# alpc91/SGRL

Hardware: AMD Instinct MI355X
Metric: env-steps/sec (whole node) + SET-actor fwd us/step, 3d_walker mix @8192 envs/GPU (higher is better)
Workload: dtype f64 (dynamics) / f32 (SET actor, obs); 1 GPU; 3D_Walker++ 8 variants x 1024 envs per GPU (config 3), random U(-1,1) actions, auto-reset, SET actor forward on every step, random-init weights; envs_per_gpu=8192, obs_max_len=287, action_max_len=21, replay_gather=none (single rank)

## Files before the change

### sgrl_amd/csrc/set_actor.hip

```cpp
#include <hip/hip_runtime.h>

#include <algorithm>
#include <cmath>
#include <cstdint>
#include <cstdlib>
#include <cstring>
#include <string>
#include <type_traits>
#include <vector>

#include "../../include/sgrl.h"
#include "../../include/sgrl_set.h"
#include "../../include/sgrl_train.h"
#include "gemm_f32.h"
#include "chain_f16.h"
#include "stream_pick.h"

namespace {

thread_local std::string g_set_err;
int sfail(int code, const std::string& msg) { g_set_err = msg; return code; }
#define SHIP_TRY(expr)                                                                     \
  do {                                                                                     \
    hipError_t _e = (expr);                                                                \
// ... 109 lines not shown
    switch (sg.kind) {
      case SGRL_PACK_COPY:
        if (i < sg.a) v = s0[i] * sg.scale;
        break;
      case SGRL_PACK_PADCOL: {
        const int r = i / sg.b, c = i % sg.b;
        if (c < sg.a) v = s0[(size_t)r * sg.a + c];
        break;
      }
      case SGRL_PACK_FOLD: {
        const int r = i / GK, k = i % GK;
        const unsigned short t = tri[k];
        if (t != 0xFFFF) {
          const int aa = t >> 8, bb = t & 255;
          const float* row = s0 + (size_t)r * (ZD * ZD);
          v = (aa == bb) ? row[aa * ZD + bb] : row[aa * ZD + bb] + row[bb * ZD + aa];
        }
        break;
      }
      case SGRL_PACK_STACK: {
        const int r = i / sg.b, c = i % sg.b;
        if (c < sg.a) {
          if (r < 30) v = s0[r * sg.a + c];
          else if (s1 && r >= 32 && r < 62) v = s1[(r - 32) * sg.a + c];
        }
        break;
      }
      case SGRL_PACK_MATMUL: {
        const int r = i / sg.b, c = i % sg.b;
        const float* ar = s0 + (size_t)r * sg.lda;
        float acc = 0.f;
        int k = 0;
        for (; k + 8 <= sg.a; k += 8) {
          float x[8], y[8];
#pragma unroll
          for (int u = 0; u < 8; u++) { x[u] = ar[k + u]; y[u] = s1[(size_t)(k + u) * sg.ldb + c]; }
#pragma unroll
          for (int u = 0; u < 8; u++) acc += x[u] * y[u];
        }
        for (; k < sg.a; k++) acc += ar[k] * s1[(size_t)k * sg.ldb + c];
        v = acc * sg.scale;
        break;
      }
      case SGRL_PACK_PERM32: {
        const int r = i / sg.a, k = i % sg.a;
        v = s0[(size_t)((r & 31) * 32 + (r >> 5)) * sg.a + k];
        break;
      }
      case SGRL_PACK_SUBMAT: {
        const int r = i / sg.b, c = i % sg.b;
        v = s0[(size_t)r * sg.lda + c];
        break;
      }
      default: break;
    }
    w[sg.dst + i] = v;
  }
}

__global__ void k_relbias(const float* rel, const float* Wr, const float* br, float* relb, const int32_t* m_off,
                          const int32_t* m_L, int n_morph) {
  const int k = blockIdx.x;
  if (k >= n_morph) return;
  const int L = m_L[k], off = m_off[k];
  for (int i = threadIdx.x; i < 2 * L * L; i += blockDim.x) {
    const int h = i / (L * L), ij = i % (L * L);
    const float* r = rel + (size_t)(off / 2) * 3 + ij * 3;
    relb[off + i] = Wr[h * 3] * r[0] + Wr[h * 3 + 1] * r[1] + Wr[h * 3 + 2] * r[2] + br[h];
  }
}

struct EnvTab {
  const int32_t* env_off;
  const int32_t* env_L;
  const int32_t* env_relb;
};
__global__ __launch_bounds__(256) void k_attention(const float* __restrict__ qkv, const float* __restrict__ U,
                                                   const float* __restrict__ gdir, const float* relb, EnvTab et,
                                                   int use_bias, const float* __restrict__ b_ng, const float* __restrict__ GD,
                                                   float* delta_dbg, float* g1, float* ng, int ng_ld,
                                                   const float* __restrict__ ln_w, const float* __restrict__ ln_b) {
  constexpr int LMAX = 14;
  __shared__ float sc[2 * LMAX * LMAX];
  __shared__ float gd[2 * LMAX * 3 * 2];
  __shared__ float dl[LMAX][128];
  const int e = blockIdx.x, t = threadIdx.x;
  const int n0 = et.env_off[e], L = et.env_L[e];
  {
    const int sub = t & 7;
    for (int idx = t >> 3; idx < 2 * L * L; idx += 32) {
      const int h = idx / (L * L), i = (idx / L) % L, j = idx % L;
      const float4* q = reinterpret_cast<const float4*>(qkv + (size_t)(n0 + i) * 768 + h * 128);
      const float4* k = reinterpret_cast<const float4*>(qkv + (size_t)(n0 + j) * 768 + 256 + h * 128);
      float s = 0.f;
#pragma unroll
      for (int u = 0; u < 4; u++) {
        const float4 a = q[sub + 8 * u], b = k[sub + 8 * u];
        s += a.x * b.x + a.y * b.y + a.z * b.z + a.w * b.w;
      }
      s += __shfl_xor(s, 1, 64); s += __shfl_xor(s, 2, 64); s += __shfl_xor(s, 4, 64);
      if (sub == 0) sc[idx] = use_bias ? s + relb[et.env_relb[e] + idx] : s;
    }
  }
  __syncthreads();
  if (t < 2 * L) {
    float* row = sc + t * L;
    float mx = row[0];
    for (int j = 1; j < L; j++) mx = fmaxf(mx, row[j]);
    float sum = 0.f;
    for (int j = 0; j < L; j++) { row[j] = expf(row[j] - mx); sum += row[j]; }
    for (int j = 0; j < L; j++) row[j] = row[j] / sum;
  }
  __syncthreads();
  for (int idx = t; idx < 2 * L * 6; idx += 256) {
    const int h = idx / (L * 6), i = (idx / 6) % L, se = idx % 6;
    const float* w = sc + (h * L + i) * L;
    float s = 0.f;
    for (int j = 0; j < L; j++) s += w[j] * gdir[(size_t)(n0 + j) * 6 + se];
    gd[idx] = s;
  }
  __syncthreads();
  {
    const int quantity = t >> 6, ln = t & 63, h = ln >> 5, c4 = (ln & 31) * 4;
    const float* vbase = quantity == 0 ? qkv + (size_t)n0 * 768 + 512 + h * 128 + c4
                                       : U + ((size_t)n0 * 3 + (quantity - 1)) * 256 + h * 128 + c4;
    auto body = [&](auto ltc, const int i0) __attribute__((always_inline)) {
      constexpr int LT = decltype(ltc)::value;
      float4 out[LT];
#pragma unroll
      for (int i = 0; i < LT; i++) out[i] = make_float4(0.f, 0.f, 0.f, 0.f);
      const float* wh = sc + h * L * L;
      if (L <= 8) {
#pragma unroll
        for (int jb = 0; jb < 8; jb += 4) {
          if (jb >= L) break;
          float4 v[4];
#pragma unroll
          for (int j = 0; j < 4; j++)
            v[j] = jb + j < L ? *reinterpret_cast<const float4*>(vbase + (size_t)(jb + j) * 768) : make_float4(0.f, 0.f, 0.f, 0.f);
#pragma unroll
          for (int j = 0; j < 4; j++)
            if (jb + j < L) {
#pragma unroll
              for (int i = 0; i < LT; i++)
                if (i0 + i < L) {
                  const float w = wh[(i0 + i) * L + jb + j];
                  out[i].x += w * v[j].x; out[i].y += w * v[j].y; out[i].z += w * v[j].z; out[i].w += w * v[j].w;
                }
            }
        }
      } else {
        float4 v = *reinterpret_cast<const float4*>(vbase);
        for (int j = 0; j < L; j++) {
          const float4 vn = *reinterpret_cast<const float4*>(vbase + (size_t)(j + 1 < L ? j + 1 : j) * 768);
#pragma unroll
          for (int i = 0; i < LT; i++)
            if (i0 + i < L) {
              const float w = wh[(i0 + i) * L + j];
              out[i].x += w * v.x; out[i].y += w * v.y; out[i].z += w * v.z; out[i].w += w * v.w;
            }
          v = vn;
        }
      }
      if (quantity != 0) {
        const float4 ga = *reinterpret_cast<const float4*>(GD + (h * 128 + c4) * 2);
        const float4 gb = *reinterpret_cast<const float4*>(GD + (h * 128 + c4) * 2 + 4);
#pragma unroll
        for (int i = 0; i < LT; i++)
          if (i0 + i < L) {
            const float* gg = gd + (h * L + i0 + i) * 6 + 2 * (quantity - 1);
            const float g0 = gg[0], g1v = gg[1];
            out[i].x += ga.x * g0 + ga.y * g1v; out[i].y += ga.z * g0 + ga.w * g1v;
            out[i].z += gb.x * g0 + gb.y * g1v; out[i].w += gb.z * g0 + gb.w * g1v;
          }
      }
      float4 bb = make_float4(0.f, 0.f, 0.f, 0.f);
      if (quantity == 0) bb = *reinterpret_cast<const float4*>(b_ng + c4);
#pragma unroll
      for (int i = 0; i < LT; i++)
        if (i0 + i < L) {
          float4 o = out[i];
          const float px = __shfl_xor(o.x, 32, 64), py = __shfl_xor(o.y, 32, 64), pz = __shfl_xor(o.z, 32, 64), pw = __shfl_xor(o.w, 32, 64);
          o = h == 0 ? make_float4(o.x + px, o.y + py, o.z + pz, o.w + pw) : make_float4(px + o.x, py + o.y, pz + o.z, pw + o.w);
          if ((i & 1) == h) {
            if (quantity != 0) {
              *reinterpret_cast<float4*>(g1 + ((size_t)(n0 + i0 + i) * 3 + (quantity - 1)) * 128 + c4) = o;
            } else {
              o.x += bb.x; o.y += bb.y; o.z += bb.z; o.w += bb.w;
              *reinterpret_cast<float4*>(&dl[i0 + i][c4]) = o;
              if (delta_dbg) *reinterpret_cast<float4*>(delta_dbg + (size_t)(n0 + i0 + i) * 128 + c4) = o;
            }
          }
        }
    };
    for (int i0 = 0; i0 < L; i0 += 4) body(std::integral_constant<int, 4>{}, i0);
  }
  __syncthreads();
  const int lane = t & 63;
  const float w0 = ln_w[lane], w1 = ln_w[64 + lane], b0 = ln_b[lane], b1 = ln_b[64 + lane];
  for (int i = t >> 6; i < L; i += 4) {
    float* row = ng + (size_t)(n0 + i) * ng_ld;
    const float v0 = row[lane] + dl[i][lane], v1 = row[64 + lane] + dl[i][64 + lane];
    const float mu = wave_sum_f32(v0 + v1) * (1.f / 128.f);
    const float d0 = v0 - mu, d1 = v1 - mu;
    const float var = wave_sum_f32(d0 * d0 + d1 * d1) * (1.f / 128.f);
    const float inv = 1.0f / sqrtf(var + 1e-5f);
    row[lane] = d0 * inv * w0 + b0;
    row[64 + lane] = d1 * inv * w1 + b1;
  }
}

__global__ __launch_bounds__(256) void k_add_ln(const float* x, int ldx, const float* delta, int ldd, const float* w,
                                                const float* b, float* out1, int ld1, float* out2, int ld2, int N) {
  const int row = blockIdx.x * 4 + (threadIdx.x >> 6), lane = threadIdx.x & 63;
  if (row >= N) return;
  float v0 = x[(size_t)row * ldx + lane], v1 = x[(size_t)row * ldx + 64 + lane];
  if (delta) { v0 += delta[(size_t)row * ldd + lane]; v1 += delta[(size_t)row * ldd + 64 + lane]; }
  const float mu = wave_sum_f32(v0 + v1) * (1.f / 128.f);
  const float d0 = v0 - mu, d1 = v1 - mu;
  const float var = wave_sum_f32(d0 * d0 + d1 * d1) * (1.f / 128.f);
  const float inv = 1.0f / sqrtf(var + 1e-5f);
  const float y0 = d0 * inv * w[lane] + b[lane], y1 = d1 * inv * w[64 + lane] + b[64 + lane];
  if (out1) { out1[(size_t)row * ld1 + lane] = y0; out1[(size_t)row * ld1 + 64 + lane] = y1; }
  if (out2) { out2[(size_t)row * ld2 + lane] = y0; out2[(size_t)row * ld2 + 64 + lane] = y1; }
}

__global__ __launch_bounds__(128) void k_equiv(const float* __restrict__ T, const float* __restrict__ W5,
                                               const float* __restrict__ g1, float* g, float* outg, int N) {
  __shared__ float Ts[8 * 96];
  const int t = threadIdx.x, n0 = blockIdx.x * 8;
  const int rows = min(8, N - n0) * 3;
  for (int o = t; o < 8 * 96; o += 128) Ts[o] = (n0 + o / 96 < N) ? T[(size_t)n0 * 96 + o] : 0.f;
  float w[32];
#pragma unroll
  for (int c = 0; c < 32; c++) w[c] = W5[t * 32 + c];
  __syncthreads();
#pragma unroll
  for (int rb = 0; rb < 24; rb += 8) {
    if (rb >= rows) break;
    float gv[8], g1v[8];
#pragma unroll
    for (int r = 0; r < 8; r++) {
      const size_t row = (size_t)n0 * 3 + (rb + r < rows ? rb + r : 0);
      gv[r] = g[row * D + t];
      g1v[r] = g1[row * D + t];
    }
#pragma unroll
    for (int r = 0; r < 8; r++) {
      if (rb + r >= rows) break;
      const float* tt = Ts + (rb + r) * 32;
      float v = 0.f;
#pragma unroll
      for (int c = 0; c < 32; c++) v += tt[c] * w[c];
      const size_t row = (size_t)n0 * 3 + rb + r;
      const float gn = gv[r] + (g1v[r] + v);
      g[row * D + t] = gn;
      if (outg) {
        outg[row * OGLD + 8 + t] = gn;
        if (t < OGLD - 136) outg[row * OGLD + 136 + t] = 0.f;
      }
    }
  }
}

__global__ __launch_bounds__(128) void k_head_out(const float* __restrict__ T, const float* __restrict__ wdec,
                                                  const float* __restrict__ obs, int obs_ld, NodeTab nt, float* act, int act_ld,
                                                  float max_action, int N) {
  const int n = blockIdx.x * 4 + (threadIdx.x >> 5), c = threadIdx.x & 31;
  if (n >= N) return;
  float vec[3];
  const float wd = wdec[c];
  for (int s = 0; s < 3; s++) {
    float v = T[(size_t)n * 96 + s * 32 + c] * wd;
    for (int off = 16; off > 0; off >>= 1) v += __shfl_xor(v, off, 32);
    vec[s] = v;
  }
  if (c < 3) {
    const int env = nt.node_env[n], limb = nt.node_limb[n];
    const float* o = obs + (size_t)env * obs_ld + 41 * limb + 3 * (5 + c);
    const float a = o[0] * vec[0] + o[1] * vec[1] + o[2] * vec[2];
    act[(size_t)env * act_ld + 3 * limb + c] = max_action * tanhf(a);
  }
}


__global__ __launch_bounds__(128) void k_head_out2(const float* __restrict__ m2, const float* __restrict__ z, const float* __restrict__ obs,
                                                   int obs_ld, NodeTab nt, float* act, int act_ld, float max_action, int N) {
  const int n = blockIdx.x * 4 + (threadIdx.x >> 5), c = threadIdx.x & 31;
  if (n >= N) return;
  float vec[3];
  const float mq = m2[(size_t)n * 32 + c];
  for (int s = 0; s < 3; s++) {
    float v = z[(size_t)n * 96 + s * 32 + c] * mq;
    for (int off = 16; off > 0; off >>= 1) v += __shfl_xor(v, off, 32);
    vec[s] = v;
  }
  if (c < 3) {
    const int env = nt.node_env[n], limb = nt.node_limb[n];
    const float* o = obs + (size_t)env * obs_ld + 41 * limb + 3 * (5 + c);
    const float a = o[0] * vec[0] + o[1] * vec[1] + o[2] * vec[2];
    act[(size_t)env * act_ld + 3 * limb + c] = max_action * tanhf(a);
  }
}

__global__ __launch_bounds__(256) void k_q_head(const float* __restrict__ c, const float* __restrict__ w, const float* __restrict__ b,
                                                const float* __restrict__ fn, NodeTab nt, float* q, int q_ld, int N) {
  const int n = blockIdx.x * 4 + (threadIdx.x >> 6), lane = threadIdx.x & 63;
  if (n >= N) return;
  const float* row = c + (size_t)n * 256;
  float v = row[lane] * w[lane] + row[64 + lane] * w[64 + lane] + row[128 + lane] * w[128 + lane] + row[192 + lane] * w[192 + lane];
  v = wave_sum_f32(v);
  if (lane == 0) q[(size_t)nt.node_env[n] * q_ld + nt.node_limb[n]] = (v + b[0]) / fn[n];
}

}

struct GraphCfg {
  std::vector<int32_t> key_i;
  std::vector<float> key_f;
  int n_env = 0, N = 0, n_morph = 0, TM = 0, Lmax = 0;
  int split_env = 0, split_node = 0;
  int32_t *d_node_env = nullptr, *d_node_limb = nullptr, *d_node_mnode = nullptr, *d_trav = nullptr;
  int32_t *d_env_off = nullptr, *d_env_L = nullptr, *d_env_relb = nullptr, *d_m_off = nullptr, *d_m_L = nullptr;
  float *d_rel = nullptr, *d_relb = nullptr;
  uint64_t last_use = 0;
  void release() {
    void* ptrs[] = {d_node_env, d_node_limb, d_node_mnode, d_trav, d_env_off, d_env_L, d_env_relb, d_m_off, d_m_L, d_rel, d_relb};
    for (void* q : ptrs) if (q) (void)hipFree(q);
  }
};

struct sgrl_set {
  const float* w = nullptr;
  int64_t off[SGRL_SET_NW];
  bool have_w = false, have_graph = false;
  int n_env = 0, N = 0, n_morph = 0, TM = 0, Lmax = 0;
  int split_env = 0, split_node = 0;
  int last_split = 0;
  int32_t *d_node_env = nullptr, *d_node_limb = nullptr, *d_node_mnode = nullptr, *d_trav = nullptr;
  int32_t *d_env_off = nullptr, *d_env_L = nullptr, *d_env_relb = nullptr, *d_m_off = nullptr, *d_m_L = nullptr;
  float *d_rel = nullptr, *d_relb = nullptr;
  std::vector<GraphCfg*> cfgs;
  uint64_t use_clock = 0;
  int64_t generation = 0;
  float* ws = nullptr;
  int64_t ws_floats = 0;
  int carved_N = 0;
  float* cat_cur = nullptr;
  float *g, *cat, *cat2, *zc, *fn, *h256, *qkv, *vg, *g1, *z2, *mat, *t256, *t256b, *t128a, *t128b, *delta,
      *outg, *outng, *gdir;
  float* wstack = nullptr;
  const float* site_ptr[SGRL_SET_NSITES];
  bool hold = false, packed_ok = false;
  int packed_form = 0;
  hipEvent_t ev_pack = nullptr;
  const float* l2mf_w = nullptr;
  const float* l2mf_b = nullptr;
  unsigned short* d_tri = nullptr;
  bool stack_dirty = true;
  bool stack_critic = false;
  int stop_after = -1;
  int small_nodes = -1;
  int gemm_form = 0;
  sgrl_gemm::EncMat* d_enc = nullptr;
  int n_enc = 0, enc_rows = 0;
  float* wsc = nullptr;
  std::vector<std::pair<int64_t, int>> enc_index;
  bool live = false;
  float* wflat = nullptr;
  unsigned* wwords = nullptr;
  int64_t wflat_floats = 0;
  sgrl_pack_seg* d_segs = nullptr;
  int2* d_chunks = nullptr;
  int n_chunks = 0;
  hipStream_t side = nullptr;
  hipEvent_t ev_fork = nullptr, ev_join = nullptr, ev_l3 = nullptr;
  hipEvent_t ev_fork_b = nullptr, ev_join_b = nullptr, ev_split = nullptr, ev_merge = nullptr;
  std::vector<hipStream_t> side_ok_for;
  int side_picks = 0;
  const float* W(int slot) const { return w + off[slot]; }
  const float* WL(int layer, int k) const { return w + off[SGRL_SET_NGLOBAL + layer * SGRL_SET_NLAYER + k]; }
};

namespace {

constexpr int64_t kPerNodeFloats = 384  + 256 + 256  + 96  + 1  + 256  + 768  +
                                   768  + 384  + 96  + 96  + 256 + 256  +
                                   128 + 128 + 128  + 3 * OGLD  + 160  + 6 ;
constexpr int kWsArrays = 19;

int64_t ws_floats_for(int64_t N) { return kPerNodeFloats * N + 32 * kWsArrays; }

void free_graphs(sgrl_set* s) {
  for (GraphCfg* c : s->cfgs) { c->release(); delete c; }
  s->cfgs.clear();
  if (s->ws) (void)hipFree(s->ws);
  s->ws = nullptr; s->ws_floats = 0; s->carved_N = 0;
  s->have_graph = false;
}

template <class T>
int upload(T** dst, const std::vector<T>& v) {
  if (hipMalloc(dst, sizeof(T) * (v.size() ? v.size() : 1)) != hipSuccess) return -1;
  if (!v.empty() && hipMemcpy(*dst, v.data(), sizeof(T) * v.size(), hipMemcpyHostToDevice) != hipSuccess) return -1;
  return 0;
}

void pick_split(const std::vector<int32_t>& env_off, int N, int* env_out, int* node_out) {
  int best = 0, best_rank = -1;
  int64_t best_dist = 0;
  for (size_t e = 1; e < env_off.size(); e++) {
    const int n = env_off[e];
    const int64_t dist = std::abs(2 * (int64_t)n - N);
    const int rank = 2 * dist > N / 16 ? 0 : (n % 128 == 0 ? 3 : n % 64 == 0 ? 2 : 1);
    if (best_rank < 0 || rank > best_rank || (rank == best_rank && dist < best_dist)) { best = (int)e; best_rank = rank; best_dist = dist; }
  }
  *env_out = best;
  *node_out = best ? env_off[best] : 0;
}

int use_cfg(sgrl_set* s, GraphCfg* c) {
  const int64_t N = c->N;
  const int64_t need = ws_floats_for(N);
  if (need > s->ws_floats) {
    if (s->ws) { (void)hipFree(s->ws); s->generation++; }
    s->ws = nullptr; s->ws_floats = 0; s->carved_N = 0;
    if (hipMalloc(&s->ws, sizeof(float) * need) != hipSuccess) return sfail(SGRL_ERR_HIP, "device allocation failed (SET workspace)");
    s->ws_floats = need;
  }
  if (s->carved_N != c->N) {
    float* p = s->ws;
    auto take = [&](int64_t n) { float* r = p; p += (n + 31) & ~int64_t(31); return r; };
    s->g = take(384 * N); s->cat = take(256 * N); s->cat2 = take(256 * N); s->zc = take(96 * N); s->fn = take(N);
    s->h256 = take(256 * N); s->qkv = take(768 * N); s->vg = take(768 * N);
    s->g1 = take(384 * N); s->z2 = take(96 * N); s->mat = take(96 * N); s->t256 = take(256 * N); s->t256b = take(256 * N); s->t128a = take(128 * N);
    s->t128b = take(128 * N); s->delta = take(128 * N); s->outg = take(3 * OGLD * N); s->outng = take(160 * N); s->gdir = take(6 * N);
    if (p - s->ws > s->ws_floats) return sfail(SGRL_ERR_LIMIT, "workspace carve-up overflow");
    s->carved_N = c->N;
  }
  s->n_env = c->n_env; s->N = c->N; s->n_morph = c->n_morph; s->TM = c->TM; s->Lmax = c->Lmax;
  s->split_env = c->split_env; s->split_node = c->split_node;
  s->d_node_env = c->d_node_env; s->d_node_limb = c->d_node_limb; s->d_node_mnode = c->d_node_mnode; s->d_trav = c->d_trav;
  s->d_env_off = c->d_env_off; s->d_env_L = c->d_env_L; s->d_env_relb = c->d_env_relb; s->d_m_off = c->d_m_off; s->d_m_L = c->d_m_L;
  s->d_rel = c->d_rel; s->d_relb = c->d_relb;
  c->last_use = ++s->use_clock;
  s->have_graph = true;
  return SGRL_OK;
}

bool gemm_use_split() {
  static const bool v = [] { const char* e = getenv("SGRL_SET_GEMM"); return !(e && e[0] == 'f'); }();
  return v;
}
struct GemmCtx {
  int form = SGRL_SET_FORM_F16X3;
  const float* w_base = nullptr; const unsigned* w_words = nullptr;
  const float* wsc = nullptr;
  const std::vector<std::pair<int64_t, int>>* enc_index = nullptr;
};
thread_local GemmCtx g_gemm;
int gemm_default_form() {
  static const int v = [] { const char* e = getenv("SGRL_SET_GEMM"); return (e && e[0] == 'b') ? SGRL_SET_FORM_BF16X6 : SGRL_SET_FORM_F16X3; }();
  return v;
}
const float* wsc_of(const float* W) {
  if (!g_gemm.enc_index) return nullptr;
  const int64_t off = W - g_gemm.w_base;
  for (const auto& e : *g_gemm.enc_index) if (e.first == off) return g_gemm.wsc + e.second;
  return nullptr;
}
GemmArgs with_words(const GemmArgs& a) {
  GemmArgs b = a;
  b.W = reinterpret_cast<const float*>(g_gemm.w_words + (a.W - g_gemm.w_base));
  b.wscale = wsc_of(a.W);
  return b;
}
template <int F> struct GemmKernels {
  static constexpr auto kNarrow = k_gemm2<F, 4, 1, 1, 2, 16, 1>;
  static constexpr auto kWide = k_gemm2<F, 4, 2, 1, 2, 32, 2>;
  static constexpr auto kSquare = k_gemm2<F, 4, 4, 1, 1, 32, 2>;
  static constexpr auto kSplit = sgrl_gemm::k_gemm3<F, 4, 2, 1, 2, 16, 2>;
  static constexpr auto kSplitH = sgrl_gemm::k_gemm3<F, 4, 2, 1, 2, 16, 2, false, false, false, 0, false, 2, true, 2>;
  static constexpr int kSplitHLds = sgrl_gemm::TileCfg3<4, 2, 1, 2, 16, 2>::kLdsBytes;
  static constexpr int kNarrowLds = sgrl_gemm::TileCfg<4, 1, 1, 2, 16>::kLdsBytes;
  static constexpr int kWideLds = sgrl_gemm::TileCfg<4, 2, 1, 2, 32>::kLdsBytes;
  static constexpr int kSquareLds = sgrl_gemm::TileCfg<4, 4, 1, 1, 32>::kLdsBytes;
  static constexpr int kSplitLds = sgrl_gemm::TileCfg3<4, 2, 1, 2, 16>::kLdsBytes;
  static bool raise_lds_limits() {
    return hipFuncSetAttribute(reinterpret_cast<const void*>(kNarrow), hipFuncAttributeMaxDynamicSharedMemorySize, kNarrowLds) == hipSuccess &&
           hipFuncSetAttribute(reinterpret_cast<const void*>(kWide), hipFuncAttributeMaxDynamicSharedMemorySize, kWideLds) == hipSuccess &&
           hipFuncSetAttribute(reinterpret_cast<const void*>(kSquare), hipFuncAttributeMaxDynamicSharedMemorySize, kSquareLds) == hipSuccess &&
           hipFuncSetAttribute(reinterpret_cast<const void*>(kSplit), hipFuncAttributeMaxDynamicSharedMemorySize, kSplitLds) == hipSuccess &&
           hipFuncSetAttribute(reinterpret_cast<const void*>(kSplitH), hipFuncAttributeMaxDynamicSharedMemorySize, kSplitHLds) == hipSuccess;
  }
  static void launch(hipStream_t st, const GemmArgs& a) {
    const int tiles128 = ((a.M + 127) / 128) * ((a.N + 127) / 128);
    if (a.N <= 64 || (a.K % 32) != 0) {
      hipLaunchKernelGGL(kNarrow, dim3(((a.M + 127) / 128) * ((a.N + 63) / 64)), dim3(256), kNarrowLds, st, a);
    } else if (gemm_use_split()) {
      if (g_gemm.form == SGRL_SET_FORM_F16X3) hipLaunchKernelGGL(kSplitH, dim3(tiles128), dim3(512), kSplitHLds, st, with_words(a));
      else hipLaunchKernelGGL(kSplit, dim3(tiles128), dim3(512), kSplitLds, st, a);
    } else if (tiles128 < 512) {
      hipLaunchKernelGGL(kNarrow, dim3(((a.M + 127) / 128) * ((a.N + 63) / 64)), dim3(256), kNarrowLds, st, a);
    } else if (a.N >= 512) {
      hipLaunchKernelGGL(kWide, dim3(tiles128), dim3(512), kWideLds, st, a);
    } else {
      hipLaunchKernelGGL(kSquare, dim3(tiles128), dim3(1024), kSquareLds, st, a);
    }
  }
};

constexpr auto kProjH = sgrl_gemm::k_gemm3<EPI_ZSPLIT, 4, 1, 1, 2, 16, 2, false, false, false, 0, false, 2, false, 2>;
constexpr int kProjHLds = sgrl_gemm::TileCfg3<4, 1, 1, 2, 16, 2>::kLdsBytes;

constexpr auto kGemmEquiv = sgrl_gemm::k_gemm3<EPI_ROWDIV | EPI_EQUIV, 4, 2, 1, 2, 16, 2>;
constexpr auto kGemmEquivH = sgrl_gemm::k_gemm3<EPI_ROWDIV | EPI_EQUIV, 4, 2, 1, 2, 16, 2, false, false, false, 0, false, 2, true, 2>;
constexpr int kEquivLds = GemmKernels<0>::kSplitLds > 128 * 100 * 4 ? GemmKernels<0>::kSplitLds : 128 * 100 * 4;
int launch_gemm_equiv(hipStream_t st, const float* A, int lda, const float* W, int ldw, const float* bias, int M, int K,
                      const float* rowdiv, const float* zq, float* tout) {
  if (K % 32 != 0 || (lda & 3) || (ldw & 3)) return sfail(SGRL_ERR_ARG, "gemm_equiv: K must be a multiple of 32 and rows 16-byte aligned");
  GemmArgs a{A, lda, W, ldw, bias, nullptr, 0, M, 1024, K, EPI_ROWDIV | EPI_EQUIV, rowdiv, nullptr, 0};
  a.zq = zq; a.tout = tout;
  if (g_gemm.form == SGRL_SET_FORM_F16X3) hipLaunchKernelGGL(kGemmEquivH, dim3(((M + 127) / 128) * 8), dim3(512), kEquivLds, st, with_words(a));
  else hipLaunchKernelGGL(kGemmEquiv, dim3(((M + 127) / 128) * 8), dim3(512), kEquivLds, st, a);
  return SGRL_OK;
}

constexpr auto kGemmGram = sgrl_gemm::k_gemm3<EPI_RELU, 4, 2, 1, 2, 16, 2, false, false, false, 0, true>;
// ... 131 lines not shown
  if (!live) return;
  float ss = 0.f;
  for (int k = lane; k < GK; k += 64) {
    const unsigned t = tri[k];
    float v = 0.f;
    if (t != 0xFFFFu) {
      const int a = t >> 8, b = t & 255;
      v = zs[w][a] * zs[w][b] + zs[w][32 + a] * zs[w][32 + b] + zs[w][64 + a] * zs[w][64 + b];
      ss += (a == b ? 1.f : 2.f) * v * v;
    }
    A[(size_t)node * GK + k] = v;
  }
  ss = wave_sum_f32(ss);
  if (lane == 0) fn[node] = sqrtf(ss) + 1.f;
}

__global__ __launch_bounds__(128) void k_zmat_perm(const float* __restrict__ zq, const float* __restrict__ matp,
                                                   float* __restrict__ tout) {
  __shared__ float ms[32 * 33], zs[96];
  const int t = threadIdx.x;
  const size_t n = blockIdx.x;
  for (int o = t; o < 1024; o += 128) ms[(o >> 5) * 33 + (o & 31)] = matp[n * 1024 + o];
  if (t < 96) zs[t] = zq[n * 96 + t];
  __syncthreads();
  if (t >= 96) return;
  const int sI = t >> 5, c = t & 31;
  float acc = 0.f;
#pragma unroll
  for (int a = 0; a < 32; a++) acc += zs[sI * 32 + a] * ms[c * 33 + a];
  tout[n * 96 + t] = acc;
}

int small_fail() { return sfail(SGRL_ERR_HIP, std::string("small-batch product: ") + sgrl_train_last_error()); }

int small_gemm(hipStream_t st, const float* A, int lda, const float* W, int ldw, const float* bias, float* C, int ldc, int M,
               int N, int K, int flags = 0, const float* rowdiv = nullptr) {
  if (flags & ~(EPI_RELU | EPI_ROWDIV)) return sfail(SGRL_ERR_ARG, "small gemm: unsupported epilogue");
  const int rc = sgrl_linear_forward(A, lda, W, ldw, bias, (flags & EPI_ROWDIV) ? rowdiv : nullptr, C, ldc, M, N, K,
                                     (flags & EPI_RELU) ? 1 : 0, st);
  return rc == SGRL_OK ? rc : small_fail();
}

int run_forward(sgrl_set* s, const float* obs, int obs_ld, float* act, int act_ld, float max_action, hipStream_t st,
                bool critic = false, const float* action = nullptr, int action_ld = 0) {
  const int N = s->N, N3 = 3 * s->N;
  const int ngf = critic ? 20 : 17;
  g_gemm.form = s->gemm_form ? s->gemm_form : gemm_default_form();
  if (!s->live || !s->wwords) g_gemm.form = SGRL_SET_FORM_BF16X6;
  if (!gemm_use_split()) g_gemm.form = SGRL_SET_FORM_BF16X6;
  g_gemm.w_base = s->w;
  g_gemm.w_words = s->wwords;
  g_gemm.wsc = s->wsc;
  g_gemm.enc_index = &s->enc_index;
  NodeTab nt{s->d_node_env, s->d_node_limb, s->d_node_mnode, s->d_trav, s->TM};
  EnvTab et{s->d_env_off, s->d_env_L, s->d_env_relb};
  const bool small = N <= (s->small_nodes >= 0 ? s->small_nodes : small_nodes());
  hipStreamCaptureStatus cap = hipStreamCaptureStatusNone;
  (void)hipStreamIsCapturing(st, &cap);
  static const bool serial_env = [] { const char* e = getenv("SGRL_SET_ONE_STREAM"); return e && e[0] == '1'; }();
  const bool one_stream = small || cap != hipStreamCaptureStatusNone || serial_env;
  if (!one_stream && sgrl_streams::enabled() && s->side_picks < 6 &&
      std::find(s->side_ok_for.begin(), s->side_ok_for.end(), st) == s->side_ok_for.end()) {
    s->side_picks++;
    hipStream_t chosen = sgrl_streams::pick({st}, s->side);
    if (chosen != s->side) s->side_ok_for.clear();
    s->side = chosen;
    s->side_ok_for.push_back(st);
  }
  hipStream_t sd = one_stream ? st : s->side;
  auto fork = [&]() { if (!one_stream) { (void)hipEventRecord(s->ev_fork, st); (void)hipStreamWaitEvent(sd, s->ev_fork, 0); } };
  auto join = [&]() { if (!one_stream) { (void)hipEventRecord(s->ev_join, sd); (void)hipStreamWaitEvent(st, s->ev_join, 0); } };
  (void)hipMemsetAsync(act, 0, sizeof(float) * (size_t)s->n_env * act_ld, st);
  const bool want_words = !small && g_gemm.form == SGRL_SET_FORM_F16X3 && gemm_use_split();
  const bool reuse = s->live && s->hold && s->packed_ok && (!want_words || s->packed_form == SGRL_SET_FORM_F16X3) && cap == hipStreamCaptureStatusNone;
  if (reuse) (void)hipStreamWaitEvent(st, s->ev_pack, 0);
  if (s->live && !reuse)
    hipLaunchKernelGGL(k_pack, dim3(s->n_chunks), dim3(256), 0, st, s->d_segs, s->d_chunks, s->d_tri, s->wflat);
  const bool encode = s->live && !reuse && want_words;
  if (encode) {
    fork();
    hipLaunchKernelGGL(sgrl_gemm::k_encode_rows, dim3((s->enc_rows + 3) / 4), dim3(256), 0, sd, s->wflat, s->wwords, s->wsc, s->d_enc, s->n_enc,
                       s->enc_rows);
  }
  hipLaunchKernelGGL(k_relbias, dim3(s->n_morph), dim3(256), 0, st, s->d_rel, s->W(SGRL_SET_REL_W), s->W(SGRL_SET_REL_B),
                     s->d_relb, s->d_m_off, s->d_m_L, s->n_morph);
  hipLaunchKernelGGL(k_embed, dim3((N + kEmbedNodes - 1) / kEmbedNodes), dim3(128), 0, st, obs, obs_ld, action, action_ld, ngf, nt,
                     s->W(SGRL_SET_GENC), s->W(SGRL_SET_ENC_W), s->W(SGRL_SET_ENC_B), s->W(SGRL_SET_EMB0), s->W(SGRL_SET_EMB1),
                     s->W(SGRL_SET_EMB2), s->g, s->cat, s->outg, s->outng, s->gdir, s->zc, s->z2, N);
  if (encode) join();
  if (s->live && !reuse && cap == hipStreamCaptureStatusNone) {
    s->packed_ok = s->hold;
    s->packed_form = want_words ? SGRL_SET_FORM_F16X3 : SGRL_SET_FORM_BF16X6;
    if (s->hold) (void)hipEventRecord(s->ev_pack, st);
  }
  const bool chain = !small && chain_enabled() && gemm_use_split() && g_gemm.form == SGRL_SET_FORM_F16X3;
  constexpr bool chain_eq = false, head_fold = true, fuse_update = true;
  struct Part {
    int r0, M, e0, ne;
    hipStream_t st, sd;
    hipEvent_t ev_fork, ev_join;
    float *catc, *cato;
    hipEvent_t ev_site0;
  };
  s->cat_cur = s->cat;
  auto site_w = [&](int site) -> const float* {
    return s->live ? s->site_ptr[site] : s->wstack + (size_t)site * 64 * 128;
  };
  if (!s->live && (s->stack_dirty || s->stack_critic != critic)) {
    s->stack_critic = critic;
    auto sw = [&](int site) { return s->wstack + (size_t)site * 64 * 128; };
    for (int l = 0; l < SGRL_SET_LAYERS; l++) {
      hipLaunchKernelGGL(k_stack_proj, dim3(32), dim3(256), 0, st, s->WL(l, SGRL_SET_A_GPROJ), (const float*)nullptr, D, D, sw(2 * l));
      hipLaunchKernelGGL(k_stack_proj, dim3(32), dim3(256), 0, st, s->WL(l, SGRL_SET_F_GPROJ2), s->WL(l, SGRL_SET_F_GPROJ3), D, D, sw(2 * l + 1));
    }
    hipLaunchKernelGGL(k_stack_proj, dim3(36), dim3(256), 0, st, s->W(SGRL_SET_GGPROJ), critic ? (const float*)nullptr : s->W(SGRL_SET_GPROJ), 136, OGLD, sw(6));
    s->stack_dirty = false;
  }
  constexpr int kStages = 4 * SGRL_SET_LAYERS + 2, kStop = 1;
  auto stage = [&](Part& p, int k) -> int {
    const int N = p.M, N3 = 3 * p.M, lnb = (N + 3) / 4;
    hipStream_t st = p.st, sd = p.sd;
    const size_t r = (size_t)p.r0;
    float *const g = s->g + 384 * r, *const zc = s->zc + 96 * r, *const z2 = s->z2 + 96 * r, *const fn = s->fn + r,
          *const h256 = s->h256 + 256 * r, *const qkv = s->qkv + 768 * r, *const vg = s->vg + 768 * r, *const g1 = s->g1 + 384 * r,
          *const mat = s->mat + 96 * r, *const t256 = s->t256 + 256 * r, *const t256b = s->t256b + 256 * r,
          *const t128a = s->t128a + 128 * r, *const t128b = s->t128b + 128 * r, *const delta = s->delta + 128 * r,
          *const outg = s->outg + 3 * OGLD * r, *const outng = s->outng + 160 * r, *const cat = s->cat + 256 * r,
          *const cat2 = s->cat2 + 256 * r;
    float *const catc = p.catc + 256 * r, *const cato = p.cato + 256 * r, *const ng = catc + 128;
    const NodeTab ntp{nt.node_env + r, nt.node_limb + r, nt.node_mnode + r, nt.trav, nt.TM};
    auto fork = [&]() { if (!one_stream && sd != st) { (void)hipEventRecord(p.ev_fork, st); (void)hipStreamWaitEvent(sd, p.ev_fork, 0); } };
    auto join = [&]() { if (!one_stream && sd != st) { (void)hipEventRecord(p.ev_join, sd); (void)hipStreamWaitEvent(st, p.ev_join, 0); } };
    int rc = SGRL_OK;
    float* const scratch = qkv;
#define G(...) do { rc = small ? small_gemm(st, __VA_ARGS__) : launch_gemm(st, __VA_ARGS__); if (rc != SGRL_OK) return rc; } while (0)
    auto gram_gemm = [&](const float* W_, const float* b_, float* C_, int ldc_, int N_) -> int {
      if (!small) return launch_gemm_gram(st, zc, W_, b_, C_, ldc_, N, N_, fn);
      hipLaunchKernelGGL(k_gram576, dim3((N + 3) / 4), dim3(256), 0, st, zc, s->d_tri, scratch, fn, N);
      return small_gemm(st, scratch, GK, W_, GK, b_, C_, ldc_, N, N_, GK, EPI_RELU);
    };
    auto equiv_gemm = [&](const float* A_, const float* W_, const float* b_) -> int {
      if (!small) return launch_gemm_equiv(st, A_, 256, W_, 256, b_, N, 256, fn, z2, mat);
      const int r_ = small_gemm(st, A_, 256, W_, 256, b_, scratch, 1024, N, 1024, 256, EPI_ROWDIV, fn);
      if (r_ != SGRL_OK) return r_;
      hipLaunchKernelGGL(k_zmat_perm, dim3(N), dim3(128), 0, st, z2, scratch, mat);
      return SGRL_OK;
    };
#define GG(W_, b_, C_, ldc_, N_) do { rc = gram_gemm(W_, b_, C_, ldc_, N_); if (rc != SGRL_OK) return rc; } while (0)
    auto pg = [&](const float* X, int ldx, int K, int site, float* z2_) -> int {
      if (K % 16 != 0 || (ldx & 3)) return sfail(SGRL_ERR_ARG, "projection: K must be a multiple of 16 and rows 16-byte aligned");
      if (small) {
        int r_ = small_gemm(st, X, ldx, site_w(site), K, nullptr, zc, ZD, N3, 30, K);
        if (r_ == SGRL_OK && z2_) r_ = small_gemm(st, X, ldx, site_w(site) + (size_t)32 * K, K, nullptr, z2_, ZD, N3, 30, K);
        return r_;
      }
      GemmArgs a{X, ldx, site_w(site), K, nullptr, zc, ZD, N3, z2_ ? 64 : 32, K, EPI_ZSPLIT, nullptr, z2_, ZD};
      if (g_gemm.form == SGRL_SET_FORM_F16X3 && gemm_use_split())
        hipLaunchKernelGGL(kProjH, dim3(((a.M + 127) / 128) * ((a.N + 63) / 64)), dim3(256), kProjHLds, st, with_words(a));
      else
        GemmKernels<EPI_ZSPLIT>::launch(st, a);
      return SGRL_OK;
    };
#define PG(...) do { rc = pg(__VA_ARGS__); if (rc != SGRL_OK) return rc; } while (0)
#define GS(...) do { rc = small ? small_gemm(sd, __VA_ARGS__) : launch_gemm(sd, __VA_ARGS__); if (rc != SGRL_OK) return rc; } while (0)
    const int l = k / 4;
    if (k < 4 * SGRL_SET_LAYERS && k % 4 == 0) {
      fork();
      GS(g, D, s->WL(l, SGRL_SET_VG_W), D, nullptr, vg, 256, N3, 256, D);
      if (chain) {
        rc = launch_site(st, g, D, D, site_w(2 * l), zc, nullptr, fn, s->WL(l, SGRL_SET_A_LG1_W), s->WL(l, SGRL_SET_A_LG1_B), 256,
                         s->WL(l, SGRL_SET_A_LG2_W), s->WL(l, SGRL_SET_A_LG2_B), catc, 256, N);
        if (rc != SGRL_OK) return rc;
        if (l == 0 && p.ev_site0) (void)hipEventRecord(p.ev_site0, st);
      } else {
        PG(g, D, D, 2 * l, nullptr);
        GG(s->WL(l, SGRL_SET_A_LG1_W), s->WL(l, SGRL_SET_A_LG1_B), h256, 256, 256);
// ... 311 lines not shown
    if (hipMalloc(&s->d_enc, sizeof(sgrl_gemm::EncMat) * mats.size()) != hipSuccess || hipMalloc(&s->wsc, sizeof(float) * rows_total) != hipSuccess ||
        hipMemcpy(s->d_enc, mats.data(), sizeof(sgrl_gemm::EncMat) * mats.size(), hipMemcpyHostToDevice) != hipSuccess)
      return sfail(SGRL_ERR_HIP, "device allocation failed in sgrl_set_bind_params (row-scale table)");
  }
  s->n_chunks = (int)chunks.size();
  s->w = s->wflat;
  std::memcpy(s->off, offsets, sizeof(int64_t) * SGRL_SET_NW);
  for (int k = 0; k < SGRL_SET_NSITES; k++) s->site_ptr[k] = s->wflat + offsets[SGRL_SET_NW + k];
  {
    std::vector<int64_t> b2(offsets, offsets + n_offsets);
    b2.push_back(total_floats);
    std::sort(b2.begin(), b2.end());
    const int64_t ow = offsets[SGRL_SET_NW + SGRL_SET_NSITES], ob = offsets[SGRL_SET_NW + SGRL_SET_NSITES + 1];
    const bool have = *std::upper_bound(b2.begin(), b2.end(), ow) - ow >= 32 * 256;
    s->l2mf_w = have ? s->wflat + ow : nullptr;
    s->l2mf_b = have ? s->wflat + ob : nullptr;
  }
  s->live = true;
  s->have_w = true;
  return SGRL_OK;
}

int sgrl_set_graph(sgrl_set* s, int n_morph, const int32_t* morph_L, const int32_t* morph_count, const int32_t* trav,
                   const float* rel) {
  if (!s || n_morph <= 0 || !morph_L || !morph_count || !trav || !rel) return sfail(SGRL_ERR_ARG, "sgrl_set_graph: bad argument");
  std::vector<int32_t> key_i;
  size_t ntrav = 0, nrel = 0;
  for (int k = 0; k < n_morph; k++) {
    if (morph_L[k] < 2 || morph_L[k] > 14) return sfail(SGRL_ERR_LIMIT, "limb count must be in [2, 14]");
    if (morph_count[k] < 0) return sfail(SGRL_ERR_ARG, "negative morph_count");
    ntrav += 3 * (size_t)morph_L[k];
    nrel += 3 * (size_t)morph_L[k] * morph_L[k];
  }
  key_i.push_back(n_morph);
  key_i.insert(key_i.end(), morph_L, morph_L + n_morph);
  key_i.insert(key_i.end(), morph_count, morph_count + n_morph);
  key_i.insert(key_i.end(), trav, trav + ntrav);
  for (GraphCfg* c : s->cfgs)
    if (c->key_i == key_i && c->key_f.size() == nrel && std::memcmp(c->key_f.data(), rel, sizeof(float) * nrel) == 0)
      return use_cfg(s, c);
  std::vector<int32_t> node_env, node_limb, node_mnode, env_off, env_L, env_relb, m_off, m_L, travT;
  int TM = 0, relb_off = 0, env = 0, node = 0, Lmax = 0;
  std::vector<int> m_node0;
  for (int k = 0; k < n_morph; k++) {
    m_node0.push_back(TM);
    m_off.push_back(relb_off);
    m_L.push_back(morph_L[k]);
    TM += morph_L[k];
    relb_off += 2 * morph_L[k] * morph_L[k];
    if (morph_L[k] > Lmax) Lmax = morph_L[k];
  }
  travT.assign(3 * (size_t)TM, 0);
  {
    size_t tp = 0;
    for (int k = 0; k < n_morph; k++) {
      const int L = morph_L[k];
      for (int q = 0; q < 3; q++)
        for (int i = 0; i < L; i++) {
          const int v = trav[tp + q * L + i];
          if (v < 0 || v >= 15) return sfail(SGRL_ERR_ARG, "traversal index out of range");
          travT[(size_t)q * TM + m_node0[k] + i] = v;
        }
      tp += 3 * (size_t)L;
    }
  }
  for (int k = 0; k < n_morph; k++) {
    for (int c = 0; c < morph_count[k]; c++) {
      env_off.push_back(node);
      env_L.push_back(morph_L[k]);
      env_relb.push_back(m_off[k]);
      for (int i = 0; i < morph_L[k]; i++) {
        node_env.push_back(env);
        node_limb.push_back(i);
        node_mnode.push_back(m_node0[k] + i);
        node++;
      }
      env++;
    }
  }
  if (node == 0) return sfail(SGRL_ERR_ARG, "no environments");
  if ((int)s->cfgs.size() >= SGRL_SET_GRAPH_CACHE) {
    size_t lru = 0;
    for (size_t i = 1; i < s->cfgs.size(); i++) if (s->cfgs[i]->last_use < s->cfgs[lru]->last_use) lru = i;
    s->cfgs[lru]->release();
    s->generation++;
    delete s->cfgs[lru];
    s->cfgs.erase(s->cfgs.begin() + lru);
  }
  GraphCfg* c = new GraphCfg();
  c->key_i = std::move(key_i);
  c->key_f.assign(rel, rel + nrel);
  c->n_env = env; c->N = node; c->n_morph = n_morph; c->TM = TM; c->Lmax = Lmax;
  pick_split(env_off, node, &c->split_env, &c->split_node);
  bool ok = upload(&c->d_node_env, node_env) == 0 && upload(&c->d_node_limb, node_limb) == 0 &&
            upload(&c->d_node_mnode, node_mnode) == 0 && upload(&c->d_trav, travT) == 0 &&
            upload(&c->d_env_off, env_off) == 0 && upload(&c->d_env_L, env_L) == 0 && upload(&c->d_env_relb, env_relb) == 0 &&
            upload(&c->d_m_off, m_off) == 0 && upload(&c->d_m_L, m_L) == 0 && upload(&c->d_rel, c->key_f) == 0;
  if (ok) ok = hipMalloc(&c->d_relb, sizeof(float) * relb_off) == hipSuccess;
  if (!ok) { c->release(); delete c; return sfail(SGRL_ERR_HIP, "device allocation failed in sgrl_set_graph"); }
  s->cfgs.push_back(c);
  return use_cfg(s, c);
}

int sgrl_set_forward(sgrl_set* s, const float* obs, int obs_ld, float* act, int act_ld, float max_action, void* stream) {
  if (!s || !obs || !act) return sfail(SGRL_ERR_ARG, "sgrl_set_forward: null argument");
  if (!s->have_w || !s->have_graph) return sfail(SGRL_ERR_ARG, "sgrl_set_forward: weights or graph not set");
  if (obs_ld < 41 * s->Lmax || act_ld < 3 * s->Lmax)
    return sfail(SGRL_ERR_ARG, "sgrl_set_forward: obs_ld < 41 * Lmax or act_ld < 3 * Lmax (rows too narrow for the largest morphology)");
  return run_forward(s, obs, obs_ld, act, act_ld, max_action, (hipStream_t)stream);
}

int sgrl_set_forward_q(sgrl_set* s, const float* obs, int obs_ld, const float* action, int action_ld, float* q, int q_ld,
                       void* stream) {
  if (!s || !obs || !action || !q) return sfail(SGRL_ERR_ARG, "sgrl_set_forward_q: null argument");
  if (!s->have_w || !s->have_graph) return sfail(SGRL_ERR_ARG, "sgrl_set_forward_q: weights or graph not set");
  if (obs_ld < 41 * s->Lmax || action_ld < 3 * s->Lmax || q_ld < s->Lmax)
    return sfail(SGRL_ERR_ARG, "sgrl_set_forward_q: obs_ld < 41 * Lmax, action_ld < 3 * Lmax or q_ld < Lmax");
  return run_forward(s, obs, obs_ld, q, q_ld, 0.f, (hipStream_t)stream, true, action, action_ld);
}

int sgrl_set_time_forward(sgrl_set* s, const float* obs, int obs_ld, float* act, int act_ld, float max_action,
                          int reps, void* stream, float* ms_out) {
  if (!s || !obs || !act || !ms_out || reps <= 0) return sfail(SGRL_ERR_ARG, "sgrl_set_time_forward: bad argument");
  if (!s->have_w || !s->have_graph) return sfail(SGRL_ERR_ARG, "weights or graph not set");
  if (obs_ld < 41 * s->Lmax || act_ld < 3 * s->Lmax) return sfail(SGRL_ERR_ARG, "sgrl_set_time_forward: rows too narrow for the largest morphology");
  hipEvent_t t0, t1;
  SHIP_TRY(hipEventCreate(&t0));
  SHIP_TRY(hipEventCreate(&t1));
  SHIP_TRY(hipEventRecord(t0, (hipStream_t)stream));
  for (int r = 0; r < reps; r++) {
    int rc = run_forward(s, obs, obs_ld, act, act_ld, max_action, (hipStream_t)stream);
    if (rc != SGRL_OK) return rc;
  }
  SHIP_TRY(hipEventRecord(t1, (hipStream_t)stream));
  SHIP_TRY(hipEventSynchronize(t1));
  float ms = 0;
  SHIP_TRY(hipEventElapsedTime(&ms, t0, t1));
  (void)hipEventDestroy(t0);
  (void)hipEventDestroy(t1);
  *ms_out = ms / reps;
  return SGRL_OK;
}

int sgrl_set_hold_weights(sgrl_set* s, int hold) {
  if (!s) return sfail(SGRL_ERR_ARG, "sgrl_set_hold_weights: null handle");
  s->hold = hold != 0;
  s->packed_ok = false;
  return SGRL_OK;
}

int sgrl_set_num_nodes(const sgrl_set* s) { return s ? s->N : SGRL_ERR_ARG; }
int64_t sgrl_set_workspace_bytes(const sgrl_set* s) { return s ? s->ws_floats * 4 : -1; }
int64_t sgrl_set_generation(const sgrl_set* s) { return s ? s->generation : -1; }
int sgrl_set_last_split(const sgrl_set* s) { return s ? s->last_split : SGRL_ERR_ARG; }

int sgrl_set_peek(sgrl_set* s, int which, float* host, int64_t n_floats) {
  if (!s || !host || !s->have_graph) return sfail(SGRL_ERR_ARG, "sgrl_set_peek: bad argument");
  const float* src[] = {s->g, s->cat_cur ? s->cat_cur : s->cat, s->zc, s->fn, s->qkv, nullptr, nullptr, s->mat, s->g1, s->delta, s->outng};
  const int64_t per[] = {384, 256, 96, 1, 768, 0, 0, 96, 384, 128, 160};
  if (which < 0 || which > 10 || !src[which] || n_floats > per[which] * s->N) return sfail(SGRL_ERR_ARG, "sgrl_set_peek: bad buffer or size");
  SHIP_TRY(hipDeviceSynchronize());
  SHIP_TRY(hipMemcpy(host, src[which], sizeof(float) * n_floats, hipMemcpyDeviceToHost));
  return SGRL_OK;
}

int sgrl_set_debug_stop_after(sgrl_set* s, int stage) {
// ... 153 lines not shown
```

Baseline: 1.932 million env-steps/s.

## Prefetch attention operands into registers and cache relative-bias across packed-weight reuse

Restructures the per-env attention kernel so that the first Q/K fragments, relative bias, gdir rows, V rows (for L<=8), the GD/bias projections and the first LayerNorm rows are all loaded up front, before the barriers. This overlaps global-load latency with the score computation. gdir is staged in shared memory instead of being re-read from global in the gd reduction. Separately, the k_relbias launch is skipped when packed weights are reused and the current graph config's relb epoch matches the pack epoch. This removes one kernel launch per step, at the cost of extra register pressure and new epoch bookkeeping that could go stale.

```diff
diff --git a/sgrl_amd/csrc/set_actor.hip b/sgrl_amd/csrc/set_actor.hip
--- a/sgrl_amd/csrc/set_actor.hip
+++ b/sgrl_amd/csrc/set_actor.hip
@@ -215,27 +215,56 @@
                                                    const float* __restrict__ ln_w, const float* __restrict__ ln_b) {
   constexpr int LMAX = 14;
   __shared__ float sc[2 * LMAX * LMAX];
+  __shared__ float gs[LMAX * 6];
   __shared__ float gd[2 * LMAX * 3 * 2];
   __shared__ float dl[LMAX][128];
   const int e = blockIdx.x, t = threadIdx.x;
-  const int n0 = et.env_off[e], L = et.env_L[e];
+  const int n0 = et.env_off[e], L = et.env_L[e], rb0 = use_bias ? et.env_relb[e] : 0;
+  const int sub = t & 7, idx0 = t >> 3, lane = t & 63;
+  const int quantity = t >> 6, h = lane >> 5, c4 = (lane & 31) * 4;
+  const float* vbase = quantity == 0 ? qkv + (size_t)n0 * 768 + 512 + h * 128 + c4
+                                     : U + ((size_t)n0 * 3 + (quantity - 1)) * 256 + h * 128 + c4;
+  float4 qa[4], kb[4];
+  float rb = 0.f;
+  if (idx0 < 2 * L * L) {
+    const int hh = idx0 / (L * L), i = (idx0 / L) % L, j = idx0 % L;
+    const float4* q = reinterpret_cast<const float4*>(qkv + (size_t)(n0 + i) * 768 + hh * 128);
+    const float4* k = reinterpret_cast<const float4*>(qkv + (size_t)(n0 + j) * 768 + 256 + hh * 128);
+#pragma unroll
+    for (int u = 0; u < 4; u++) { qa[u] = q[sub + 8 * u]; kb[u] = k[sub + 8 * u]; }
+    if (use_bias) rb = relb[rb0 + idx0];
+  }
+  float gdv = 0.f;
+  if (t < 6 * L) gdv = gdir[(size_t)n0 * 6 + t];
+  float4 v8[8];
   {
-    const int sub = t & 7;
-    for (int idx = t >> 3; idx < 2 * L * L; idx += 32) {
-      const int h = idx / (L * L), i = (idx / L) % L, j = idx % L;
-      const float4* q = reinterpret_cast<const float4*>(qkv + (size_t)(n0 + i) * 768 + h * 128);
-      const float4* k = reinterpret_cast<const float4*>(qkv + (size_t)(n0 + j) * 768 + 256 + h * 128);
-      float s = 0.f;
-#pragma unroll
-      for (int u = 0; u < 4; u++) {
-        const float4 a = q[sub + 8 * u], b = k[sub + 8 * u];
-        s += a.x * b.x + a.y * b.y + a.z * b.z + a.w * b.w;
-      }
-      s += __shfl_xor(s, 1, 64); s += __shfl_xor(s, 2, 64); s += __shfl_xor(s, 4, 64);
-      if (sub == 0) sc[idx] = use_bias ? s + relb[et.env_relb[e] + idx] : s;
-    }
-  }
+    const int held = L <= 8 ? L : 1;
+#pragma unroll
+    for (int j = 0; j < 8; j++)
+      if (j < held) v8[j] = *reinterpret_cast<const float4*>(vbase + (size_t)j * 768);
+  }
+  for (int idx = idx0; idx < 2 * L * L; idx += 32) {
+    if (idx != idx0) {
+      const int hh = idx / (L * L), i = (idx / L) % L, j = idx % L;
+      const float4* q = reinterpret_cast<const float4*>(qkv + (size_t)(n0 + i) * 768 + hh * 128);
+      const float4* k = reinterpret_cast<const float4*>(qkv + (size_t)(n0 + j) * 768 + 256 + hh * 128);
+#pragma unroll
+      for (int u = 0; u < 4; u++) { qa[u] = q[sub + 8 * u]; kb[u] = k[sub + 8 * u]; }
+      if (use_bias) rb = relb[rb0 + idx];
+    }
+    float s = 0.f;
+#pragma unroll
+    for (int u = 0; u < 4; u++) {
+      const float4 a = qa[u], b = kb[u];
+      s += a.x * b.x + a.y * b.y + a.z * b.z + a.w * b.w;
+    }
+    s += __shfl_xor(s, 1, 64); s += __shfl_xor(s, 2, 64); s += __shfl_xor(s, 4, 64);
+    if (sub == 0) sc[idx] = use_bias ? s + rb : s;
+  }
+  if (t < 6 * L) gs[t] = gdv;
   __syncthreads();
+  const float4 pa = quantity == 0 ? *reinterpret_cast<const float4*>(b_ng + c4) : *reinterpret_cast<const float4*>(GD + (h * 128 + c4) * 2);
+  const float4 pb = quantity == 0 ? make_float4(0.f, 0.f, 0.f, 0.f) : *reinterpret_cast<const float4*>(GD + (h * 128 + c4) * 2 + 4);
   if (t < 2 * L) {
     float* row = sc + t * L;
     float mx = row[0];
@@ -246,71 +275,28 @@
   }
   __syncthreads();
   for (int idx = t; idx < 2 * L * 6; idx += 256) {
-    const int h = idx / (L * 6), i = (idx / 6) % L, se = idx % 6;
-    const float* w = sc + (h * L + i) * L;
+    const int hh = idx / (L * 6), i = (idx / 6) % L, se = idx % 6;
+    const float* w = sc + (hh * L + i) * L;
     float s = 0.f;
-    for (int j = 0; j < L; j++) s += w[j] * gdir[(size_t)(n0 + j) * 6 + se];
+    for (int j = 0; j < L; j++) s += w[j] * gs[j * 6 + se];
     gd[idx] = s;
   }
   __syncthreads();
   {
-    const int quantity = t >> 6, ln = t & 63, h = ln >> 5, c4 = (ln & 31) * 4;
-    const float* vbase = quantity == 0 ? qkv + (size_t)n0 * 768 + 512 + h * 128 + c4
-                                       : U + ((size_t)n0 * 3 + (quantity - 1)) * 256 + h * 128 + c4;
-    auto body = [&](auto ltc, const int i0) __attribute__((always_inline)) {
-      constexpr int LT = decltype(ltc)::value;
-      float4 out[LT];
-#pragma unroll
-      for (int i = 0; i < LT; i++) out[i] = make_float4(0.f, 0.f, 0.f, 0.f);
-      const float* wh = sc + h * L * L;
-      if (L <= 8) {
-#pragma unroll
-        for (int jb = 0; jb < 8; jb += 4) {
-          if (jb >= L) break;
-          float4 v[4];
-#pragma unroll
-          for (int j = 0; j < 4; j++)
-            v[j] = jb + j < L ? *reinterpret_cast<const float4*>(vbase + (size_t)(jb + j) * 768) : make_float4(0.f, 0.f, 0.f, 0.f);
-#pragma unroll
-          for (int j = 0; j < 4; j++)
-            if (jb + j < L) {
-#pragma unroll
-              for (int i = 0; i < LT; i++)
-                if (i0 + i < L) {
-                  const float w = wh[(i0 + i) * L + jb + j];
-                  out[i].x += w * v[j].x; out[i].y += w * v[j].y; out[i].z += w * v[j].z; out[i].w += w * v[j].w;
-                }
-            }
-        }
-      } else {
-        float4 v = *reinterpret_cast<const float4*>(vbase);
-        for (int j = 0; j < L; j++) {
-          const float4 vn = *reinterpret_cast<const float4*>(vbase + (size_t)(j + 1 < L ? j + 1 : j) * 768);
-#pragma unroll
-          for (int i = 0; i < LT; i++)
-            if (i0 + i < L) {
-              const float w = wh[(i0 + i) * L + j];
-              out[i].x += w * v.x; out[i].y += w * v.y; out[i].z += w * v.z; out[i].w += w * v.w;
-            }
-          v = vn;
-        }
-      }
+    const float* wh = sc + h * L * L;
+    auto finish = [&](float4 (&out)[4], const int i0) __attribute__((always_inline)) {
       if (quantity != 0) {
-        const float4 ga = *reinterpret_cast<const float4*>(GD + (h * 128 + c4) * 2);
-        const float4 gb = *reinterpret_cast<const float4*>(GD + (h * 128 + c4) * 2 + 4);
-#pragma unroll
-        for (int i = 0; i < LT; i++)
+#pragma unroll
+        for (int i = 0; i < 4; i++)
           if (i0 + i < L) {
             const float* gg = gd + (h * L + i0 + i) * 6 + 2 * (quantity - 1);
             const float g0 = gg[0], g1v = gg[1];
-            out[i].x += ga.x * g0 + ga.y * g1v; out[i].y += ga.z * g0 + ga.w * g1v;
-            out[i].z += gb.x * g0 + gb.y * g1v; out[i].w += gb.z * g0 + gb.w * g1v;
+            out[i].x += pa.x * g0 + pa.y * g1v; out[i].y += pa.z * g0 + pa.w * g1v;
+            out[i].z += pb.x * g0 + pb.y * g1v; out[i].w += pb.z * g0 + pb.w * g1v;
           }
       }
-      float4 bb = make_float4(0.f, 0.f, 0.f, 0.f);
-      if (quantity == 0) bb = *reinterpret_cast<const float4*>(b_ng + c4);
-#pragma unroll
-      for (int i = 0; i < LT; i++)
+#pragma unroll
+      for (int i = 0; i < 4; i++)
         if (i0 + i < L) {
           float4 o = out[i];
           const float px = __shfl_xor(o.x, 32, 64), py = __shfl_xor(o.y, 32, 64), pz = __shfl_xor(o.z, 32, 64), pw = __shfl_xor(o.w, 32, 64);
@@ -319,27 +305,75 @@
             if (quantity != 0) {
               *reinterpret_cast<float4*>(g1 + ((size_t)(n0 + i0 + i) * 3 + (quantity - 1)) * 128 + c4) = o;
             } else {
-              o.x += bb.x; o.y += bb.y; o.z += bb.z; o.w += bb.w;
+              o.x += pa.x; o.y += pa.y; o.z += pa.z; o.w += pa.w;
               *reinterpret_cast<float4*>(&dl[i0 + i][c4]) = o;
               if (delta_dbg) *reinterpret_cast<float4*>(delta_dbg + (size_t)(n0 + i0 + i) * 128 + c4) = o;
             }
           }
         }
     };
-    for (int i0 = 0; i0 < L; i0 += 4) body(std::integral_constant<int, 4>{}, i0);
+    if (L <= 8) {
+      for (int i0 = 0; i0 < L; i0 += 4) {
+        float4 out[4];
+#pragma unroll
+        for (int i = 0; i < 4; i++) out[i] = make_float4(0.f, 0.f, 0.f, 0.f);
+#pragma unroll
+        for (int j = 0; j < 8; j++)
+          if (j < L) {
+#pragma unroll
+            for (int i = 0; i < 4; i++)
+              if (i0 + i < L) {
+                const float w = wh[(i0 + i) * L + j];
+                out[i].x += w * v8[j].x; out[i].y += w * v8[j].y; out[i].z += w * v8[j].z; out[i].w += w * v8[j].w;
+              }
+          }
+        finish(out, i0);
+      }
+    } else {
+      for (int i0 = 0; i0 < L; i0 += 4) {
+        float4 out[4];
+#pragma unroll
+        for (int i = 0; i < 4; i++) out[i] = make_float4(0.f, 0.f, 0.f, 0.f);
+        float4 v = v8[0];
+        for (int j = 0; j < L; j++) {
+          const float4 vn = *reinterpret_cast<const float4*>(vbase + (size_t)(j + 1 < L ? j + 1 : j) * 768);
+#pragma unroll
+          for (int i = 0; i < 4; i++)
+            if (i0 + i < L) {
+              const float w = wh[(i0 + i) * L + j];
+              out[i].x += w * v.x; out[i].y += w * v.y; out[i].z += w * v.z; out[i].w += w * v.w;
+            }
+          v = vn;
+        }
+        finish(out, i0);
+      }
+    }
   }
   __syncthreads();
-  const int lane = t & 63;
+  float x0[2] = {0.f, 0.f}, x1[2] = {0.f, 0.f};
+#pragma unroll
+  for (int r = 0; r < 2; r++)
+    if (quantity + 4 * r < L) {
+      const float* row = ng + (size_t)(n0 + quantity + 4 * r) * ng_ld;
+      x0[r] = row[lane]; x1[r] = row[64 + lane];
+    }
   const float w0 = ln_w[lane], w1 = ln_w[64 + lane], b0 = ln_b[lane], b1 = ln_b[64 + lane];
-  for (int i = t >> 6; i < L; i += 4) {
+  auto ln_row = [&](const int i, const float xa, const float xb) __attribute__((always_inline)) {
     float* row = ng + (size_t)(n0 + i) * ng_ld;
-    const float v0 = row[lane] + dl[i][lane], v1 = row[64 + lane] + dl[i][64 + lane];
+    const float v0 = xa + dl[i][lane], v1 = xb + dl[i][64 + lane];
     const float mu = wave_sum_f32(v0 + v1) * (1.f / 128.f);
     const float d0 = v0 - mu, d1 = v1 - mu;
     const float var = wave_sum_f32(d0 * d0 + d1 * d1) * (1.f / 128.f);
     const float inv = 1.0f / sqrtf(var + 1e-5f);
     row[lane] = d0 * inv * w0 + b0;
     row[64 + lane] = d1 * inv * w1 + b1;
+  };
+#pragma unroll
+  for (int r = 0; r < 2; r++)
+    if (quantity + 4 * r < L) ln_row(quantity + 4 * r, x0[r], x1[r]);
+  for (int i = quantity + 8; i < L; i += 4) {
+    const float* row = ng + (size_t)(n0 + i) * ng_ld;
+    ln_row(i, row[lane], row[64 + lane]);
   }
 }
 
@@ -456,6 +490,7 @@
   int32_t *d_node_env = nullptr, *d_node_limb = nullptr, *d_node_mnode = nullptr, *d_trav = nullptr;
   int32_t *d_env_off = nullptr, *d_env_L = nullptr, *d_env_relb = nullptr, *d_m_off = nullptr, *d_m_L = nullptr;
   float *d_rel = nullptr, *d_relb = nullptr;
+  uint64_t relb_epoch = 0;
   uint64_t last_use = 0;
   void release() {
     void* ptrs[] = {d_node_env, d_node_limb, d_node_mnode, d_trav, d_env_off, d_env_L, d_env_relb, d_m_off, d_m_L, d_rel, d_relb};
@@ -474,6 +509,7 @@
   int32_t *d_env_off = nullptr, *d_env_L = nullptr, *d_env_relb = nullptr, *d_m_off = nullptr, *d_m_L = nullptr;
   float *d_rel = nullptr, *d_relb = nullptr;
   std::vector<GraphCfg*> cfgs;
+  GraphCfg* cur = nullptr;
   uint64_t use_clock = 0;
   int64_t generation = 0;
   float* ws = nullptr;
@@ -486,6 +522,7 @@
   const float* site_ptr[SGRL_SET_NSITES];
   bool hold = false, packed_ok = false;
   int packed_form = 0;
+  uint64_t pack_epoch = 0;
   hipEvent_t ev_pack = nullptr;
   const float* l2mf_w = nullptr;
   const float* l2mf_b = nullptr;
@@ -530,6 +567,7 @@
   if (s->ws) (void)hipFree(s->ws);
   s->ws = nullptr; s->ws_floats = 0; s->carved_N = 0;
   s->have_graph = false;
+  s->cur = nullptr;
 }
 
 template <class T>
@@ -577,6 +615,7 @@
   s->d_env_off = c->d_env_off; s->d_env_L = c->d_env_L; s->d_env_relb = c->d_env_relb; s->d_m_off = c->d_m_off; s->d_m_L = c->d_m_L;
   s->d_rel = c->d_rel; s->d_relb = c->d_relb;
   c->last_use = ++s->use_clock;
+  s->cur = c;
   s->have_graph = true;
   return SGRL_OK;
 }
@@ -874,8 +913,10 @@
     hipLaunchKernelGGL(sgrl_gemm::k_encode_rows, dim3((s->enc_rows + 3) / 4), dim3(256), 0, sd, s->wflat, s->wwords, s->wsc, s->d_enc, s->n_enc,
                        s->enc_rows);
   }
-  hipLaunchKernelGGL(k_relbias, dim3(s->n_morph), dim3(256), 0, st, s->d_rel, s->W(SGRL_SET_REL_W), s->W(SGRL_SET_REL_B),
-                     s->d_relb, s->d_m_off, s->d_m_L, s->n_morph);
+  const bool relb_ok = reuse && s->cur && s->cur->relb_epoch == s->pack_epoch;
+  if (!relb_ok)
+    hipLaunchKernelGGL(k_relbias, dim3(s->n_morph), dim3(256), 0, st, s->d_rel, s->W(SGRL_SET_REL_W), s->W(SGRL_SET_REL_B),
+                       s->d_relb, s->d_m_off, s->d_m_L, s->n_morph);
   hipLaunchKernelGGL(k_embed, dim3((N + kEmbedNodes - 1) / kEmbedNodes), dim3(128), 0, st, obs, obs_ld, action, action_ld, ngf, nt,
                      s->W(SGRL_SET_GENC), s->W(SGRL_SET_ENC_W), s->W(SGRL_SET_ENC_B), s->W(SGRL_SET_EMB0), s->W(SGRL_SET_EMB1),
                      s->W(SGRL_SET_EMB2), s->g, s->cat, s->outg, s->outng, s->gdir, s->zc, s->z2, N);
@@ -883,7 +924,11 @@
   if (s->live && !reuse && cap == hipStreamCaptureStatusNone) {
     s->packed_ok = s->hold;
     s->packed_form = want_words ? SGRL_SET_FORM_F16X3 : SGRL_SET_FORM_BF16X6;
-    if (s->hold) (void)hipEventRecord(s->ev_pack, st);
+    s->pack_epoch++;
+  }
+  if (s->live && s->hold && !relb_ok && cap == hipStreamCaptureStatusNone) {
+    if (s->cur) s->cur->relb_epoch = s->pack_epoch;
+    (void)hipEventRecord(s->ev_pack, st);
   }
   const bool chain = !small && chain_enabled() && gemm_use_split() && g_gemm.form == SGRL_SET_FORM_F16X3;
   constexpr bool chain_eq = false, head_fold = true, fuse_update = true;
@@ -1361,6 +1406,7 @@
   if ((int)s->cfgs.size() >= SGRL_SET_GRAPH_CACHE) {
     size_t lru = 0;
     for (size_t i = 1; i < s->cfgs.size(); i++) if (s->cfgs[i]->last_use < s->cfgs[lru]->last_use) lru = i;
+    if (s->cur == s->cfgs[lru]) s->cur = nullptr;
     s->cfgs[lru]->release();
     s->generation++;
     delete s->cfgs[lru];
```

After: 1.927 million env-steps/s. Within noise of the previous version (-0.2%).
